# awkrail/svpc

Measured on AMD Instinct MI355X. Metric: train steps/sec (vivt, batch=16, clip_seq=12), higher is better.
Workload: dtype bf16x3; 1 GPU; MODEL_TYPE=vivt train step: N=16 videos/GPU x S=12 clips x Lv=100 frames x F=3072, Lt=22, D=768, H=12, L=6 (enc+step-enc+dec), V=951, A=384, E=10; dropout .1/.1/.4; fwd+bwd+allreduce+clip+BertAdam; mode=bf16x3, global_batch=16, parallelism=dp1, launch=hipGraph replay, gpus_requested=1

## Files before the change

svpc_amd/csrc/layernorm.hip:

```cpp
#include "common.h"
#include <stdlib.h>

template <int W, typename T>
struct VecIO;
template <>
struct VecIO<4, float> {
    static __device__ __forceinline__ void load(const float* p, float* v) {
        float4 t = *reinterpret_cast<const float4*>(p);
        v[0] = t.x; v[1] = t.y; v[2] = t.z; v[3] = t.w;
    }
    static __device__ __forceinline__ void store(float* p, const float* v) {
        *reinterpret_cast<float4*>(p) = make_float4(v[0], v[1], v[2], v[3]);
    }
};
template <>
struct VecIO<1, float> {
    static __device__ __forceinline__ void load(const float* p, float* v) { v[0] = p[0]; }
    static __device__ __forceinline__ void store(float* p, const float* v) { p[0] = v[0]; }
};
typedef __bf16 bf16x4_t __attribute__((ext_vector_type(4)));
template <>
struct VecIO<4, __bf16> {
    static __device__ __forceinline__ void load(const __bf16* p, float* v) {
        bf16x4_t t = *reinterpret_cast<const bf16x4_t*>(p);
        v[0] = (float)t[0]; v[1] = (float)t[1]; v[2] = (float)t[2]; v[3] = (float)t[3];
    }
    static __device__ __forceinline__ void store(__bf16* p, const float* v) {
        bf16x4_t t;
        t[0] = (__bf16)v[0]; t[1] = (__bf16)v[1]; t[2] = (__bf16)v[2]; t[3] = (__bf16)v[3];
        *reinterpret_cast<bf16x4_t*>(p) = t;
    }
};
template <>
struct VecIO<1, __bf16> {
    static __device__ __forceinline__ void load(const __bf16* p, float* v) { v[0] = (float)p[0]; }
    static __device__ __forceinline__ void store(__bf16* p, const float* v) { p[0] = (__bf16)v[0]; }
};

struct split16 { __bf16 v; };
template <>
struct VecIO<4, split16> {
    static __device__ __forceinline__ void load2(const split16* p, int lo, float* v) {
        const bf16x4_t h = *reinterpret_cast<const bf16x4_t*>(p), l = *reinterpret_cast<const bf16x4_t*>(p + lo);
#pragma unroll
        for (int j = 0; j < 4; ++j) v[j] = (float)h[j] + (float)l[j];
    }
    static __device__ __forceinline__ void store2(split16* p, int lo, const float* v) {
        bf16x4_t h, l;
#pragma unroll
        for (int j = 0; j < 4; ++j) { h[j] = (__bf16)v[j]; l[j] = (__bf16)(v[j] - (float)h[j]); }
        *reinterpret_cast<bf16x4_t*>(p) = h;
        *reinterpret_cast<bf16x4_t*>(p + lo) = l;
    }
};
template <>
struct VecIO<1, split16> {
    static __device__ __forceinline__ void load2(const split16* p, int lo, float* v) { v[0] = (float)p[0].v + (float)p[lo].v; }
    static __device__ __forceinline__ void store2(split16* p, int lo, const float* v) {
        const __bf16 h = (__bf16)v[0];
        p[0].v = h; p[lo].v = (__bf16)(v[0] - (float)h);
    }
};
template <typename T> struct IsSplit { static constexpr bool value = false; };
template <> struct IsSplit<split16> { static constexpr bool value = true; };
template <int W, typename T> __device__ __forceinline__ void ln_load(const T* p, int lo, float* v) {
    if constexpr (IsSplit<T>::value) VecIO<W, T>::load2(p, lo, v); else VecIO<W, T>::load(p, v);
}
template <int W, typename T> __device__ __forceinline__ void ln_store(T* p, int lo, const float* v) {
    if constexpr (IsSplit<T>::value) VecIO<W, T>::store2(p, lo, v); else VecIO<W, T>::store(p, v);
}

struct LnArgs {
    const void* x; const int* src_rows; const void* res; const float* gamma; const float* beta;
    void* y; float* mean; float* rstd; int R; int D; float eps;
    float p_pre; uint32_t site_pre; float p_post; uint32_t site_post; const u64* seed;
    const float* add1; int mod1; const float* add2; const int* idx2;
    int ldx, ldr, ldy;
    int lox, lor, loy;
};

template <int NPL, int W, typename TX, typename TY>
__global__ __launch_bounds__(256) void ln_fwd_kernel(LnArgs a) {
    const TX* __restrict__ xp = reinterpret_cast<const TX*>(a.x);
    const TY* __restrict__ rp = reinterpret_cast<const TY*>(a.res);
    TY* __restrict__ yp = reinterpret_cast<TY*>(a.y);
    const int lane = threadIdx.x & 63;
    const int r = __builtin_amdgcn_readfirstlane(blockIdx.x * 4 + (threadIdx.x >> 6));
    if (r >= a.R) return;
    const int D = a.D;
    const size_t xrow = (size_t)(a.src_rows ? a.src_rows[r] : r) * a.ldx;
    const size_t orow = (size_t)r * D;
    const size_t rrow = (size_t)r * a.ldr, yrow = (size_t)r * a.ldy;
    const bool any_drop = (a.p_pre > 0.f) || (a.p_post > 0.f);
    const u64 seed = any_drop ? a.seed[0] : 0ull;
    const float ik_pre = a.p_pre > 0.f ? 1.0f / (1.0f - a.p_pre) : 1.0f;
    const float ik_post = a.p_post > 0.f ? 1.0f / (1.0f - a.p_post) : 1.0f;

    float v[NPL * W];
    float sum = 0.f;
    const bool full = D == NPL * W * 64;
    if (full) {
#pragma unroll
        for (int i = 0; i < NPL; ++i) ln_load<W, TX>(xp + xrow + (lane + 64 * i) * W, a.lox, &v[i * W]);
        if constexpr (NPL * W <= 16) {
            float t[NPL * W];
            if (a.res) {
#pragma unroll
                for (int i = 0; i < NPL; ++i) ln_load<W, TY>(rp + rrow + (lane + 64 * i) * W, a.lor, &t[i * W]);
            }
            if (a.p_pre > 0.f) {
#pragma unroll
                for (int k = 0; k < NPL * W; ++k)
                    v[k] *= drop_scale(seed, a.site_pre, orow + (lane + 64 * (k / W)) * W + (k % W), a.p_pre, ik_pre);
            }
            if (a.res) {
#pragma unroll
                for (int k = 0; k < NPL * W; ++k) v[k] += t[k];
            }
        } else {
            if (a.p_pre > 0.f) {
#pragma unroll
                for (int k = 0; k < NPL * W; ++k)
                    v[k] *= drop_scale(seed, a.site_pre, orow + (lane + 64 * (k / W)) * W + (k % W), a.p_pre, ik_pre);
            }
            if (a.res) {
#pragma unroll
                for (int i = 0; i < NPL; ++i) {
                    float t[W];
                    ln_load<W, TY>(rp + rrow + (lane + 64 * i) * W, a.lor, t);
#pragma unroll
                    for (int j = 0; j < W; ++j) v[i * W + j] += t[j];
                }
            }
        }
#pragma unroll
        for (int k = 0; k < NPL * W; ++k) sum += v[k];
    }
#pragma unroll
    for (int i = 0; i < NPL; ++i) {
        if (full) break;
        const int col = (lane + 64 * i) * W;
        if (col < D) {
            ln_load<W, TX>(xp + xrow + col, a.lox, &v[i * W]);
            if (a.p_pre > 0.f) {
#pragma unroll
                for (int j = 0; j < W; ++j) v[i * W + j] *= drop_scale(seed, a.site_pre, orow + col + j, a.p_pre, ik_pre);
            }
            if (a.res) {
                float t[W];
                ln_load<W, TY>(rp + rrow + col, a.lor, t);
#pragma unroll
                for (int j = 0; j < W; ++j) v[i * W + j] += t[j];
            }
#pragma unroll
            for (int j = 0; j < W; ++j) sum += v[i * W + j];
        }
    }
    const float mean = wave_sum(sum) / (float)D;
    float sq = 0.f;
#pragma unroll
    for (int i = 0; i < NPL; ++i) {
        const int col = (lane + 64 * i) * W;
        if (col < D) {
#pragma unroll
            for (int j = 0; j < W; ++j) {
                float d = v[i * W + j] - mean;
                sq += d * d;
            }
        }
    }
    const float var = wave_sum(sq) / (float)D;
    const float rstd = 1.0f / sqrtf(var + a.eps);
    if (lane == 0) {
        if (a.mean) a.mean[r] = mean;
        if (a.rstd) a.rstd[r] = rstd;
    }
    const size_t a1row = a.add1 ? (size_t)(r % a.mod1) * D : 0;
    const size_t a2row = a.add2 ? (size_t)a.idx2[r] * D : 0;
    if (full) {
        constexpr int CH = NPL < 4 ? NPL : (NPL > 8 ? 2 : 4);
#pragma unroll
        for (int i0 = 0; i0 < NPL; i0 += CH) {
            float g[CH][W], b[CH][W], t1[CH][W], t2[CH][W];
#pragma unroll
            for (int c = 0; c < CH; ++c) {
                if (i0 + c < NPL) {
                    const int col = (lane + 64 * (i0 + c)) * W;
                    VecIO<W, float>::load(a.gamma + col, g[c]);
                    VecIO<W, float>::load(a.beta + col, b[c]);
                }
            }
            if (a.add1) {
#pragma unroll
                for (int c = 0; c < CH; ++c)
                    if (i0 + c < NPL) VecIO<W, float>::load(a.add1 + a1row + (lane + 64 * (i0 + c)) * W, t1[c]);
            }
            if (a.add2) {
#pragma unroll
                for (int c = 0; c < CH; ++c)
                    if (i0 + c < NPL) VecIO<W, float>::load(a.add2 + a2row + (lane + 64 * (i0 + c)) * W, t2[c]);
            }
#pragma unroll
            for (int c = 0; c < CH; ++c) {
                if (i0 + c < NPL) {
                    const int i = i0 + c, col = (lane + 64 * i) * W;
                    float o[W];
#pragma unroll
                    for (int j = 0; j < W; ++j) {
                        float t = (v[i * W + j] - mean) * rstd * g[c][j] + b[c][j];
                        if (a.p_post > 0.f) t *= drop_scale(seed, a.site_post, orow + col + j, a.p_post, ik_post);
                        if (a.add1) t += t1[c][j];
                        if (a.add2) t += t2[c][j];
                        o[j] = t;
                    }
                    ln_store<W, TY>(yp + yrow + col, a.loy, o);
                }
            }
        }
        return;
    }
#pragma unroll
    for (int i = 0; i < NPL; ++i) {
        const int col = (lane + 64 * i) * W;
        if (col < D) {
            float g[W], b[W], o[W];
            VecIO<W, float>::load(a.gamma + col, g);
            VecIO<W, float>::load(a.beta + col, b);
#pragma unroll
            for (int j = 0; j < W; ++j) {
                float t = (v[i * W + j] - mean) * rstd * g[j] + b[j];
                if (a.p_post > 0.f) t *= drop_scale(seed, a.site_post, orow + col + j, a.p_post, ik_post);
                o[j] = t;
            }
            if (a.add1) {
                float t[W];
                VecIO<W, float>::load(a.add1 + a1row + col, t);
#pragma unroll
                for (int j = 0; j < W; ++j) o[j] += t[j];
            }
            if (a.add2) {
                float t[W];
                VecIO<W, float>::load(a.add2 + a2row + col, t);
#pragma unroll
                for (int j = 0; j < W; ++j) o[j] += t[j];
            }
            ln_store<W, TY>(yp + yrow + col, a.loy, o);
        }
    }
}

constexpr int LNW_NPL = 6;
template <typename TX, typename TY>
__global__ __launch_bounds__(256) void ln_fwd_wide_kernel(LnArgs a, int rows_per_wg) {
    __shared__ float gb[2][3072];
    __shared__ float red[2][4];
    const TX* __restrict__ xp = reinterpret_cast<const TX*>(a.x);
    TY* __restrict__ yp = reinterpret_cast<TY*>(a.y);
    const int lane = threadIdx.x & 63, wave = __builtin_amdgcn_readfirstlane(threadIdx.x >> 6);
    const int pair = wave >> 1, half = wave & 1;
    const int D = a.D;
    const int r0 = blockIdx.x * rows_per_wg, r1 = min(a.R, r0 + rows_per_wg);
    const int iters = (r1 - r0 + 1) >> 1;
    const int cbase = (half * LNW_NPL * 64 + lane) * 4;
    const u64 seed = a.p_post > 0.f ? a.seed[0] : 0ull;
    const float ik_post = a.p_post > 0.f ? 1.0f / (1.0f - a.p_post) : 1.0f;
    auto src = [&](int r) { return (size_t)(a.src_rows ? a.src_rows[r] : r) * a.ldx; };
    float v[LNW_NPL * 4], nx[LNW_NPL * 4];
    {
        const size_t xrow = src(min(r0 + pair, r1 - 1));
#pragma unroll
        for (int i = 0; i < LNW_NPL; ++i) ln_load<4, TX>(xp + xrow + cbase + 256 * i, a.lox, &nx[i * 4]);
    }
    for (int c = threadIdx.x * 4; c < D; c += 1024) {
        *reinterpret_cast<float4*>(&gb[0][c]) = *reinterpret_cast<const float4*>(a.gamma + c);
        *reinterpret_cast<float4*>(&gb[1][c]) = *reinterpret_cast<const float4*>(a.beta + c);
    }
    for (int it = 0; it < iters; ++it) {
        const int rr = r0 + 2 * it + pair;
        const bool ok = rr < r1;
        const int r = min(rr, r1 - 1);
#pragma unroll
        for (int k = 0; k < LNW_NPL * 4; ++k) v[k] = nx[k];
        if (it + 1 < iters) {
            const size_t xrow = src(min(rr + 2, r1 - 1));
#pragma unroll
            for (int i = 0; i < LNW_NPL; ++i) ln_load<4, TX>(xp + xrow + cbase + 256 * i, a.lox, &nx[i * 4]);
        }
        float sum = 0.f;
#pragma unroll
        for (int k = 0; k < LNW_NPL * 4; ++k) sum += v[k];
        sum = wave_sum(sum);
        if (lane == 0) red[0][wave] = sum;
        __syncthreads();
        const float mean = (red[0][pair * 2] + red[0][pair * 2 + 1]) / (float)D;
        float sq = 0.f;
#pragma unroll
        for (int k = 0; k < LNW_NPL * 4; ++k) { const float d = v[k] - mean; sq += d * d; }
        sq = wave_sum(sq);
        if (lane == 0) red[1][wave] = sq;
        __syncthreads();
        const float var = (red[1][pair * 2] + red[1][pair * 2 + 1]) / (float)D;
        const float rstd = 1.0f / sqrtf(var + a.eps);
        if (ok && half == 0 && lane == 0) {
            if (a.mean) a.mean[r] = mean;
            if (a.rstd) a.rstd[r] = rstd;
        }
        if (ok) {
            const size_t orow = (size_t)r * D, yrow = (size_t)r * a.ldy;
#pragma unroll
            for (int i = 0; i < LNW_NPL; ++i) {
                const int col = cbase + 256 * i;
                const float4 g = *reinterpret_cast<const float4*>(&gb[0][col]), b = *reinterpret_cast<const float4*>(&gb[1][col]);
                const float gg[4] = {g.x, g.y, g.z, g.w}, bb[4] = {b.x, b.y, b.z, b.w};
                float o[4];
#pragma unroll
                for (int j = 0; j < 4; ++j) {
                    float t = (v[i * 4 + j] - mean) * rstd * gg[j] + bb[j];
                    if (a.p_post > 0.f) t *= drop_scale(seed, a.site_post, orow + col + j, a.p_post, ik_post);
                    o[j] = t;
                }
                ln_store<4, TY>(yp + yrow + col, a.loy, o);
            }
        }
    }
}

struct LnBwdArgs {
    const void* dy; const void* x; const int* src_rows; const void* res; const float* gamma;
    const float* mean; const float* rstd;
    void* dh;
    void* dx;
    float* partial;
    int R; int D;
    float p_pre; uint32_t site_pre; float p_post; uint32_t site_post; const u64* seed;
    int ldx, ldr;
};

template <int NPL, int W, typename TX, typename TY, int RU>
__global__ __launch_bounds__(256, (W == 4 && NPL * W <= 12 && RU == 2) ? 4 : 1) void ln_bwd_kernel(LnBwdArgs a) {
    constexpr bool LACC = W == 4 && NPL * W <= 12 && RU == 2;
    extern __shared__ float smem[];
    const TY* __restrict__ dyp = reinterpret_cast<const TY*>(a.dy);
    const TX* __restrict__ xp = reinterpret_cast<const TX*>(a.x);
    const TY* __restrict__ rp = reinterpret_cast<const TY*>(a.res);
    TY* __restrict__ dhp = reinterpret_cast<TY*>(a.dh);
    TX* __restrict__ dxp = reinterpret_cast<TX*>(a.dx);
    const int lane = threadIdx.x & 63;
    const int wave = __builtin_amdgcn_readfirstlane(threadIdx.x >> 6);
    const int D = a.D;
    const bool any_drop = (a.p_pre > 0.f) || (a.p_post > 0.f);
    const u64 seed = any_drop ? a.seed[0] : 0ull;
    const float ik_pre = a.p_pre > 0.f ? 1.0f / (1.0f - a.p_pre) : 1.0f;
    const float ik_post = a.p_post > 0.f ? 1.0f / (1.0f - a.p_post) : 1.0f;
    const float invD = 1.0f / (float)D;

    float g[LACC ? 1 : NPL * W], accg[LACC ? 1 : NPL * W], accb[LACC ? 1 : NPL * W];
    float* const lg = smem;
    float* const lacc = smem + D + (size_t)wave * 2 * D;
    if constexpr (LACC) {
#pragma unroll
        for (int i = 0; i < NPL; ++i) {
            const int col = (lane + 64 * i) * W;
            if (col < D) {
                *reinterpret_cast<float4*>(lacc + col) = make_float4(0.f, 0.f, 0.f, 0.f);
                *reinterpret_cast<float4*>(lacc + D + col) = make_float4(0.f, 0.f, 0.f, 0.f);
                if (wave == 0) *reinterpret_cast<float4*>(lg + col) = *reinterpret_cast<const float4*>(a.gamma + col);
            }
        }
        __syncthreads();
    } else {
#pragma unroll
        for (int i = 0; i < NPL; ++i) {
            const int col = (lane + 64 * i) * W;
#pragma unroll
            for (int j = 0; j < W; ++j) { accg[i * W + j] = 0.f; accb[i * W + j] = 0.f; g[i * W + j] = 0.f; }
            if (col < D) VecIO<W, float>::load(a.gamma + col, &g[i * W]);
        }
    }
    const int stride = gridDim.x * 4;
    for (int r0 = blockIdx.x * 4 + wave; r0 < a.R; r0 += stride * RU) {
        float h[RU][NPL * W], d[RU][NPL * W];
        float mean[RU], rstd[RU];
        const bool full = D == NPL * W * 64;
#pragma unroll
        for (int u = 0; u < RU; ++u) {
            const int r = r0 + u * stride;
            if (r < a.R) {
                const size_t xrow = (size_t)(a.src_rows ? a.src_rows[r] : r) * a.ldx;
                const size_t orow = (size_t)r * D, rrow = (size_t)r * a.ldr;
                mean[u] = a.mean[r]; rstd[u] = a.rstd[r];
                if (full) {
                    float t[NPL * W];
#pragma unroll
                    for (int i = 0; i < NPL; ++i) VecIO<W, TX>::load(xp + xrow + (lane + 64 * i) * W, &h[u][i * W]);
#pragma unroll
                    for (int i = 0; i < NPL; ++i) VecIO<W, TY>::load(dyp + orow + (lane + 64 * i) * W, &d[u][i * W]);
                    if (a.res) {
#pragma unroll
                        for (int i = 0; i < NPL; ++i) VecIO<W, TY>::load(rp + rrow + (lane + 64 * i) * W, &t[i * W]);
                    }
                    if (a.p_pre > 0.f) {
#pragma unroll
                        for (int i = 0; i < NPL; ++i)
#pragma unroll
                            for (int j = 0; j < W; ++j)
                                h[u][i * W + j] *= drop_scale(seed, a.site_pre, orow + (lane + 64 * i) * W + j, a.p_pre, ik_pre);
                    }
                    if (a.res) {
#pragma unroll
                        for (int k = 0; k < NPL * W; ++k) h[u][k] += t[k];
                    }
                    continue;
                }
#pragma unroll
                for (int i = 0; i < NPL; ++i) {
                    const int col = (lane + 64 * i) * W;
                    if (col < D) {
                        VecIO<W, TX>::load(xp + xrow + col, &h[u][i * W]);
                        VecIO<W, TY>::load(dyp + orow + col, &d[u][i * W]);
                        if (a.res) {
                            float t[W];
                            VecIO<W, TY>::load(rp + rrow + col, t);
                            if (a.p_pre > 0.f) {
#pragma unroll
                                for (int j = 0; j < W; ++j)
                                    h[u][i * W + j] *= drop_scale(seed, a.site_pre, orow + col + j, a.p_pre, ik_pre);
                            }
#pragma unroll
                            for (int j = 0; j < W; ++j) h[u][i * W + j] += t[j];
                        } else if (a.p_pre > 0.f) {
#pragma unroll
                            for (int j = 0; j < W; ++j) h[u][i * W + j] *= drop_scale(seed, a.site_pre, orow + col + j, a.p_pre, ik_pre);
                        }
                    }
                }
            }
        }
#pragma unroll
        for (int u = 0; u < RU; ++u) {
            const int r = r0 + u * stride;
            if (r >= a.R) continue;
            const size_t orow = (size_t)r * D;
            float s1 = 0.f, s2 = 0.f;
#pragma unroll
            for (int i = 0; i < NPL; ++i) {
                const int col = (lane + 64 * i) * W;
                if (col < D) {
                    float gv[W], ag[W], ab[W];
                    if constexpr (LACC) {
                        const float4 t0 = *reinterpret_cast<const float4*>(lg + col), t1 = *reinterpret_cast<const float4*>(lacc + col),
                                     t2 = *reinterpret_cast<const float4*>(lacc + D + col);
                        gv[0] = t0.x; gv[1] = t0.y; gv[2] = t0.z; gv[3] = t0.w;
                        ag[0] = t1.x; ag[1] = t1.y; ag[2] = t1.z; ag[3] = t1.w;
                        ab[0] = t2.x; ab[1] = t2.y; ab[2] = t2.z; ab[3] = t2.w;
                    }
#pragma unroll
                    for (int j = 0; j < W; ++j) {
                        float dy0 = d[u][i * W + j];
                        if (a.p_post > 0.f) dy0 *= drop_scale(seed, a.site_post, orow + col + j, a.p_post, ik_post);
                        const float xhat = (h[u][i * W + j] - mean[u]) * rstd[u];
                        if constexpr (LACC) { ag[j] += dy0 * xhat; ab[j] += dy0; }
                        else { accg[i * W + j] += dy0 * xhat; accb[i * W + j] += dy0; }
                        const float t = dy0 * (LACC ? gv[j] : g[i * W + j]);
                        h[u][i * W + j] = xhat;
                        d[u][i * W + j] = t;
                        s1 += t;
                        s2 += t * xhat;
                    }
                    if constexpr (LACC) {
                        *reinterpret_cast<float4*>(lacc + col) = make_float4(ag[0], ag[1], ag[2], ag[3]);
                        *reinterpret_cast<float4*>(lacc + D + col) = make_float4(ab[0], ab[1], ab[2], ab[3]);
                    }
                }
            }
            if (a.dh || a.dx) {
                s1 = wave_sum(s1) * invD;
                s2 = wave_sum(s2) * invD;
                if (full) {
                    float o[NPL * W];
#pragma unroll
                    for (int k = 0; k < NPL * W; ++k) o[k] = rstd[u] * (d[u][k] - s1 - h[u][k] * s2);
                    if (a.dh) {
#pragma unroll
                        for (int i = 0; i < NPL; ++i) VecIO<W, TY>::store(dhp + orow + (lane + 64 * i) * W, &o[i * W]);
                    }
                    if (a.dx && a.dx != a.dh) {
                        if (a.p_pre > 0.f) {
#pragma unroll
                            for (int k = 0; k < NPL * W; ++k)
                                o[k] *= drop_scale(seed, a.site_pre, orow + (lane + 64 * (k / W)) * W + (k % W), a.p_pre, ik_pre);
                        }
#pragma unroll
                        for (int i = 0; i < NPL; ++i) VecIO<W, TX>::store(dxp + orow + (lane + 64 * i) * W, &o[i * W]);
                    }
                    continue;
                }
#pragma unroll
                for (int i = 0; i < NPL; ++i) {
                    const int col = (lane + 64 * i) * W;
                    if (col < D) {
                        float o[W];
#pragma unroll
                        for (int j = 0; j < W; ++j) o[j] = rstd[u] * (d[u][i * W + j] - s1 - h[u][i * W + j] * s2);
                        if (a.dh) VecIO<W, TY>::store(dhp + orow + col, o);
                        if (a.dx && a.dx != a.dh) {
                            if (a.p_pre > 0.f) {
#pragma unroll
                                for (int j = 0; j < W; ++j) o[j] *= drop_scale(seed, a.site_pre, orow + col + j, a.p_pre, ik_pre);
                            }
                            VecIO<W, TX>::store(dxp + orow + col, o);
                        }
                    }
                }
            }
        }
    }
    if constexpr (LACC) {
        __syncthreads();
        float* out = a.partial + (size_t)blockIdx.x * 2 * D;
        for (int c = threadIdx.x; c < 2 * D; c += 256) {
            float v = smem[D + c];
#pragma unroll
            for (int w = 1; w < 4; ++w) v += smem[D + (size_t)w * 2 * D + c];
            out[c] = v;
        }
        return;
    }
#pragma unroll
    for (int w = 0; w < 4; ++w) {
        if (wave == w) {
#pragma unroll
            for (int i = 0; i < NPL; ++i) {
                const int col = (lane + 64 * i) * W;
                if (col < D) {
#pragma unroll
                    for (int j = 0; j < W; ++j) {
                        if (w == 0) { smem[col + j] = accg[i * W + j]; smem[D + col + j] = accb[i * W + j]; }
                        else { smem[col + j] += accg[i * W + j]; smem[D + col + j] += accb[i * W + j]; }
                    }
                }
            }
        }
        __syncthreads();
    }
    float* out = a.partial + (size_t)blockIdx.x * 2 * D;
    for (int c = threadIdx.x; c < 2 * D; c += 256) out[c] = smem[c];
}

template <typename TX, typename TY>
__global__ __launch_bounds__(256) void ln_param_grad_kernel(LnBwdArgs a, int rows_per_group) {
    __shared__ float red[4][2][256];
    const TY* __restrict__ dyp = reinterpret_cast<const TY*>(a.dy);
    const TX* __restrict__ xp = reinterpret_cast<const TX*>(a.x);
    const TY* __restrict__ rp = reinterpret_cast<const TY*>(a.res);
    const int cg = threadIdx.x & 63, rl = threadIdx.x >> 6, D = a.D;
    const int c0 = (blockIdx.x * 64 + cg) * 4;
    const int group = blockIdx.y;
    const int r0 = group * rows_per_group, r1 = min(a.R, r0 + rows_per_group);
    const bool any_drop = (a.p_pre > 0.f) || (a.p_post > 0.f);
    const u64 seed = any_drop ? a.seed[0] : 0ull;
    const float ik_pre = a.p_pre > 0.f ? 1.0f / (1.0f - a.p_pre) : 1.0f;
    const float ik_post = a.p_post > 0.f ? 1.0f / (1.0f - a.p_post) : 1.0f;
    float ag[4] = {0.f, 0.f, 0.f, 0.f}, ab[4] = {0.f, 0.f, 0.f, 0.f};
    auto one = [&](int r, const float* h, const float* d, const float* t, float mean, float rstd) {
        const size_t orow = (size_t)r * D;
#pragma unroll
        for (int j = 0; j < 4; ++j) {
            float hv = h[j];
            if (a.p_pre > 0.f) hv *= drop_scale(seed, a.site_pre, orow + c0 + j, a.p_pre, ik_pre);
            if (a.res) hv += t[j];
            float dy0 = d[j];
            if (a.p_post > 0.f) dy0 *= drop_scale(seed, a.site_post, orow + c0 + j, a.p_post, ik_post);
            ag[j] += dy0 * (hv - mean) * rstd;
            ab[j] += dy0;
        }
    };
    if (c0 < D) {
        int r = r0 + rl;
        for (; r + 12 < r1; r += 16) {
            float h4[4][4], d4[4][4], t4[4][4];
            float m4[4], s4[4];
#pragma unroll
            for (int q = 0; q < 4; ++q) {
                const int rq = r + 4 * q;
                VecIO<4, TX>::load(xp + (size_t)(a.src_rows ? a.src_rows[rq] : rq) * a.ldx + c0, h4[q]);
                VecIO<4, TY>::load(dyp + (size_t)rq * D + c0, d4[q]);
                if (a.res) VecIO<4, TY>::load(rp + (size_t)rq * a.ldr + c0, t4[q]);
                else { t4[q][0] = t4[q][1] = t4[q][2] = t4[q][3] = 0.f; }
                m4[q] = a.mean[rq]; s4[q] = a.rstd[rq];
            }
#pragma unroll
            for (int q = 0; q < 4; ++q) one(r + 4 * q, h4[q], d4[q], t4[q], m4[q], s4[q]);
        }
        for (; r + 4 < r1; r += 8) {
            const int ra = r, rb = r + 4;
            float ha[4], hb[4], da[4], db[4], ta[4] = {0.f, 0.f, 0.f, 0.f}, tb[4] = {0.f, 0.f, 0.f, 0.f};
            VecIO<4, TX>::load(xp + (size_t)(a.src_rows ? a.src_rows[ra] : ra) * a.ldx + c0, ha);
            VecIO<4, TX>::load(xp + (size_t)(a.src_rows ? a.src_rows[rb] : rb) * a.ldx + c0, hb);
            VecIO<4, TY>::load(dyp + (size_t)ra * D + c0, da);
            VecIO<4, TY>::load(dyp + (size_t)rb * D + c0, db);
            if (a.res) { VecIO<4, TY>::load(rp + (size_t)ra * a.ldr + c0, ta); VecIO<4, TY>::load(rp + (size_t)rb * a.ldr + c0, tb); }
            const float ma = a.mean[ra], sa = a.rstd[ra], mb = a.mean[rb], sb = a.rstd[rb];
            one(ra, ha, da, ta, ma, sa);
            one(rb, hb, db, tb, mb, sb);
        }
        for (; r < r1; r += 4) {
            float h[4], d[4], t[4] = {0.f, 0.f, 0.f, 0.f};
            VecIO<4, TX>::load(xp + (size_t)(a.src_rows ? a.src_rows[r] : r) * a.ldx + c0, h);
            VecIO<4, TY>::load(dyp + (size_t)r * D + c0, d);
            if (a.res) VecIO<4, TY>::load(rp + (size_t)r * a.ldr + c0, t);
            one(r, h, d, t, a.mean[r], a.rstd[r]);
        }
    }
#pragma unroll
    for (int j = 0; j < 4; ++j) { red[rl][0][cg * 4 + j] = ag[j]; red[rl][1][cg * 4 + j] = ab[j]; }
    __syncthreads();
    float* out = a.partial + (size_t)group * 2 * D;
    const int i = threadIdx.x, c = blockIdx.x * 256 + i;
    if (c < D) {
        out[c] = (red[0][0][i] + red[1][0][i]) + (red[2][0][i] + red[3][0][i]);
        out[D + c] = (red[0][1][i] + red[1][1][i]) + (red[2][1][i] + red[3][1][i]);
    }
}

__device__ __forceinline__ float finalize_column(const float* __restrict__ partial, int G, int ncols, int c, int rg, float (*red)[33]) {
    const int cl = threadIdx.x & 31;
    float s = 0.f;
    if (c < ncols) {
        int g = rg;
        for (; g + 224 < G; g += 256) {
            float a[8];
#pragma unroll
            for (int k = 0; k < 8; ++k) a[k] = partial[(size_t)(g + 32 * k) * ncols + c];
#pragma unroll
            for (int k = 0; k < 8; ++k) s += a[k];
        }
        for (; g + 96 < G; g += 128) {
            const float a0 = partial[(size_t)g * ncols + c], a1 = partial[(size_t)(g + 32) * ncols + c];
            const float a2 = partial[(size_t)(g + 64) * ncols + c], a3 = partial[(size_t)(g + 96) * ncols + c];
            s += a0; s += a1; s += a2; s += a3;
        }
        for (; g < G; g += 32) s += partial[(size_t)g * ncols + c];
    }
    red[rg][cl] = s;
    __syncthreads();
    float t = 0.f;
    if (rg == 0) {
        t = red[0][cl];
#pragma unroll
        for (int k = 1; k < 32; ++k) t += red[k][cl];
    }
    return t;
}
__global__ __launch_bounds__(1024) void colsum_finalize_kernel(const float* __restrict__ partial, int G, int ncols,
                                                               float* __restrict__ out, int accumulate) {
    __shared__ float red[32][33];
    const int cl = threadIdx.x & 31, rg = threadIdx.x >> 5;
    const int c = blockIdx.x * 32 + cl;
    const float t = finalize_column(partial, G, ncols, c, rg, red);
    if (rg == 0 && c < ncols) out[c] = accumulate ? out[c] + t : t;
}

__global__ __launch_bounds__(1024) void ln_finalize_kernel(const float* __restrict__ partial, int G, int D, float* __restrict__ dgamma,
                                                           float* __restrict__ dbeta, int accumulate) {
    __shared__ float red[32][33];
    const int cl = threadIdx.x & 31, rg = threadIdx.x >> 5;
    const int c = blockIdx.x * 32 + cl, ncols = 2 * D;
    const float t = finalize_column(partial, G, ncols, c, rg, red);
    if (rg == 0 && c < ncols) {
        float* out = c < D ? dgamma + c : dbeta + (c - D);
        *out = accumulate ? *out + t : t;
    }
}

struct FEntry { const float* partial; float* out0; float* out1; int groups, ncols, split, block0; };
constexpr int FIN_MAX = 64;
struct FArgs { int n; FEntry e[FIN_MAX]; };

__global__ __launch_bounds__(1024) void multi_finalize_kernel(FArgs a) {
    __shared__ float red[32][33];
    int ei = 0;
    while (ei + 1 < a.n && (int)blockIdx.x >= a.e[ei + 1].block0) ++ei;
    const FEntry& en = a.e[ei];
    const int cl = threadIdx.x & 31, rg = threadIdx.x >> 5;
    const int c = ((int)blockIdx.x - en.block0) * 32 + cl;
    const float t = finalize_column(en.partial, en.groups, en.ncols, c, rg, red);
    if (rg == 0 && c < en.ncols) {
        float* out = c < en.split ? en.out0 + c : en.out1 + (c - en.split);
        *out += t;
    }
}

template <int KMAX, typename T>
__global__ __launch_bounds__(256) void bucket_colsum_kernel(const T* __restrict__ x, int ldx, const int* __restrict__ idx,
                                                            int R, int C, int K, int rows_per_chunk, float* __restrict__ partial) {
    const int c = blockIdx.x * 256 + threadIdx.x;
    const int chunk = blockIdx.y;
    const int r0 = chunk * rows_per_chunk;
    const int r1 = min(R, r0 + rows_per_chunk);
    float acc[KMAX];
#pragma unroll
    for (int k = 0; k < KMAX; ++k) acc[k] = 0.f;
    if (c < C) {
        for (int r = r0; r < r1; ++r) {
            const float v = (float)x[(size_t)r * ldx + c];
            const int k = idx ? idx[r] : 0;
#pragma unroll
            for (int kk = 0; kk < KMAX; ++kk) acc[kk] += (kk == k) ? v : 0.f;
        }
#pragma unroll
        for (int k = 0; k < KMAX; ++k)
            if (k < K) partial[((size_t)chunk * K + k) * C + c] = acc[k];
    }
}

template <typename T>
__device__ __forceinline__ void colsum_vec_block(float (*red)[512], const T* __restrict__ x, int ldx, int R, int C, int rows_per_chunk,
                                                 float* __restrict__ partial, int colblock, int chunk) {
    constexpr int V = 16 / sizeof(T);
    typedef float vec16 __attribute__((ext_vector_type(4)));
    typedef __bf16 bf16x8v __attribute__((ext_vector_type(8)));
    const int cg = threadIdx.x & 63, rl = threadIdx.x >> 6;
    const int c0 = (colblock * 64 + cg) * V;
    const int r0 = chunk * rows_per_chunk, r1 = min(R, r0 + rows_per_chunk);
    float acc[V];
#pragma unroll
    for (int j = 0; j < V; ++j) acc[j] = 0.f;
    auto add = [&](const vec16& raw) {
        if (sizeof(T) == 4) {
#pragma unroll
            for (int j = 0; j < 4; ++j) acc[j] += raw[j];
        } else {
            union { vec16 f; bf16x8v h; } u;
            u.f = raw;
#pragma unroll
            for (int j = 0; j < 8; ++j) acc[j % V] += (float)u.h[j];
        }
    };
    if (c0 < C) {
        int r = r0 + rl;
        for (; r + 12 < r1; r += 16) {
            const vec16 a0 = *reinterpret_cast<const vec16*>(x + (size_t)r * ldx + c0);
            const vec16 a1 = *reinterpret_cast<const vec16*>(x + (size_t)(r + 4) * ldx + c0);
            const vec16 a2 = *reinterpret_cast<const vec16*>(x + (size_t)(r + 8) * ldx + c0);
            const vec16 a3 = *reinterpret_cast<const vec16*>(x + (size_t)(r + 12) * ldx + c0);
            add(a0); add(a1); add(a2); add(a3);
        }
        for (; r < r1; r += 4) add(*reinterpret_cast<const vec16*>(x + (size_t)r * ldx + c0));
    }
#pragma unroll
    for (int j = 0; j < V; ++j) red[rl][cg * V + j] = acc[j];
    __syncthreads();
    for (int i = threadIdx.x; i < 64 * V; i += 256) {
        const int c = colblock * 64 * V + i;
        if (c < C) partial[(size_t)chunk * C + c] = (red[0][i] + red[1][i]) + (red[2][i] + red[3][i]);
    }
}

template <typename T>
__global__ __launch_bounds__(256) void colsum_vec_kernel(const T* __restrict__ x, int ldx, int R, int C, int rows_per_chunk,
                                                         float* __restrict__ partial) {
    __shared__ float red[4][512];
    colsum_vec_block<T>(red, x, ldx, R, C, rows_per_chunk, partial, blockIdx.x, blockIdx.y);
}

struct CEntry { const void* x; float* partial; int dt, ldx, R, C, rpc, colblocks, block0; };
constexpr int CSUM_MAX = 48;
struct CArgs { int n; CEntry e[CSUM_MAX]; };
__global__ __launch_bounds__(256) void multi_colsum_kernel(CArgs a) {
    __shared__ float red[4][512];
    int ei = 0;
    while (ei + 1 < a.n && (int)blockIdx.x >= a.e[ei + 1].block0) ++ei;
    const CEntry& en = a.e[ei];
    const int local = blockIdx.x - en.block0;
    const int colblock = local % en.colblocks, chunk = local / en.colblocks;
    if (en.dt == 0) colsum_vec_block<float>(red, (const float*)en.x, en.ldx, en.R, en.C, en.rpc, en.partial, colblock, chunk);
    else colsum_vec_block<__bf16>(red, (const __bf16*)en.x, en.ldx, en.R, en.C, en.rpc, en.partial, colblock, chunk);
}

template <int NPL, int W>
static int launch_ln_fwd(const LnArgs& a, int x_dt, int y_dt, hipStream_t s) {
    const dim3 g(ceil_div(a.R, 4)), b(256);
    if (x_dt == 0 && y_dt == 0) hipLaunchKernelGGL((ln_fwd_kernel<NPL, W, float, float>), g, b, 0, s, a);
    else if (x_dt == 0 && y_dt == 1) hipLaunchKernelGGL((ln_fwd_kernel<NPL, W, float, __bf16>), g, b, 0, s, a);
    else if (x_dt == 1 && y_dt == 1) hipLaunchKernelGGL((ln_fwd_kernel<NPL, W, __bf16, __bf16>), g, b, 0, s, a);
    else if (x_dt == 0 && y_dt == 2) hipLaunchKernelGGL((ln_fwd_kernel<NPL, W, float, split16>), g, b, 0, s, a);
    else if (x_dt == 2 && y_dt == 2) hipLaunchKernelGGL((ln_fwd_kernel<NPL, W, split16, split16>), g, b, 0, s, a);
    else if (x_dt == 2 && y_dt == 0) hipLaunchKernelGGL((ln_fwd_kernel<NPL, W, split16, float>), g, b, 0, s, a);
    else { svpc_set_error("ln_fwd: storage-type combination not instantiated"); return -1; }
    return svpc_check_launch("ln_fwd");
}
template <int NPL, int W>
static int launch_ln_bwd(const LnBwdArgs& a, int G, int x_dt, int y_dt, hipStream_t s) {
    const dim3 g(G), b(256);
    constexpr int RU = (NPL * W <= 16) ? 2 : 1;
    constexpr bool LACC = W == 4 && NPL * W <= 12 && RU == 2;
    static int ru_env = -1;
    if (ru_env < 0) { const char* e = getenv("SVPC_LN_RU"); ru_env = e ? atoi(e) : 0; }
    const size_t lds = (size_t)((LACC && ru_env != 1) ? 9 : 2) * a.D * sizeof(float);
    if (ru_env == 1) {
        if (x_dt == 0 && y_dt == 0) hipLaunchKernelGGL((ln_bwd_kernel<NPL, W, float, float, 1>), g, b, lds, s, a);
        else if (x_dt == 0 && y_dt == 1) hipLaunchKernelGGL((ln_bwd_kernel<NPL, W, float, __bf16, 1>), g, b, lds, s, a);
        else hipLaunchKernelGGL((ln_bwd_kernel<NPL, W, __bf16, __bf16, 1>), g, b, lds, s, a);
        return svpc_check_launch("ln_bwd");
    }
    if (x_dt == 0 && y_dt == 0) hipLaunchKernelGGL((ln_bwd_kernel<NPL, W, float, float, RU>), g, b, lds, s, a);
    else if (x_dt == 0 && y_dt == 1) hipLaunchKernelGGL((ln_bwd_kernel<NPL, W, float, __bf16, RU>), g, b, lds, s, a);
    else hipLaunchKernelGGL((ln_bwd_kernel<NPL, W, __bf16, __bf16, RU>), g, b, lds, s, a);
    return svpc_check_launch("ln_bwd");
}

static bool aligned16(const void* p) { return (((uintptr_t)p) & 15) == 0; }
extern "C" int svpc_ln_param_only_groups(int R);

extern "C" {

int svpc_ln_fwd_s(const void* x, int x_dt, int ldx, int lox, const int* src_rows, const void* res, int ldr, int lor, const float* gamma,
                  const float* beta, void* y, int y_dt, int ldy, int loy, float* mean, float* rstd, int R, int D, float eps, float p_pre,
                  unsigned site_pre, float p_post, unsigned site_post, const u64* seed, const float* add1, int mod1, const float* add2,
                  const int* idx2, hipStream_t stream) {
    if (R == 0) return 0;
    SVPC_REQUIRE(!(x_dt == 1 && y_dt == 0), "ln_fwd: bf16 input with fp32 output is not instantiated");
    if (ldx <= 0) ldx = D;
    if (ldr <= 0) ldr = D;
    if (ldy <= 0) ldy = D;
    SVPC_REQUIRE((x_dt != 2 || (lox >= D && ldx >= lox + D)) && (y_dt != 2 || (loy >= D && ldy >= loy + D && (!res || (lor >= D && ldr >= lor + D)))),
                 "ln_fwd: a split tensor needs its lo plane inside the row, behind the hi plane");
    LnArgs a{x, src_rows, res, gamma, beta, y, mean, rstd, R, D, eps, p_pre, site_pre, p_post, site_post, seed,
             add1, mod1, add2, idx2, ldx, ldr, ldy, lox, lor, loy};
    SVPC_REQUIRE((p_pre <= 0.f && p_post <= 0.f) || seed != nullptr, "ln_fwd: dropout needs a seed pointer");
    const bool vec = (D % 4 == 0) && aligned16(x) && aligned16(y) && aligned16(gamma) && aligned16(beta) &&
                     (!res || aligned16(res)) && (!add1 || aligned16(add1)) && (!add2 || aligned16(add2)) &&
                     ldx % 4 == 0 && ldy % 4 == 0 && ldr % 4 == 0 && lox % 4 == 0 && lor % 4 == 0 && loy % 4 == 0;
    if (vec) {
        if (D <= 256) return launch_ln_fwd<1, 4>(a, x_dt, y_dt, stream);
        static int npl3 = -1;
        if (npl3 < 0) { const char* e = getenv("SVPC_LN_FWD_NPL3"); npl3 = e ? atoi(e) : 1; }
        if (D <= 768 && npl3) return launch_ln_fwd<3, 4>(a, x_dt, y_dt, stream);
        if (D <= 1024) return launch_ln_fwd<4, 4>(a, x_dt, y_dt, stream);
        static int wide = -1;
        if (wide < 0) { const char* e = getenv("SVPC_LN_WIDE"); wide = e ? atoi(e) : 1; }
        if (wide && D == 3072 && x_dt == 0 && !res && p_pre <= 0.f && !add1 && !add2) {
            int rpw = ceil_div(R, 1280);
            rpw += rpw & 1;
            const dim3 g(ceil_div(R, rpw)), b(256);
            if (y_dt == 2) hipLaunchKernelGGL((ln_fwd_wide_kernel<float, split16>), g, b, 0, stream, a, rpw);
            else if (y_dt == 1) hipLaunchKernelGGL((ln_fwd_wide_kernel<float, __bf16>), g, b, 0, stream, a, rpw);
            else hipLaunchKernelGGL((ln_fwd_wide_kernel<float, float>), g, b, 0, stream, a, rpw);
            return svpc_check_launch("ln_fwd_wide");
        }
        if (D <= 3072) return launch_ln_fwd<12, 4>(a, x_dt, y_dt, stream);
        if (D <= 8192) return launch_ln_fwd<32, 4>(a, x_dt, y_dt, stream);
    } else {
        if (D <= 256) return launch_ln_fwd<4, 1>(a, x_dt, y_dt, stream);
        if (D <= 1024) return launch_ln_fwd<16, 1>(a, x_dt, y_dt, stream);
        if (D <= 3072) return launch_ln_fwd<48, 1>(a, x_dt, y_dt, stream);
    }
    svpc_set_error("ln_fwd: row width not supported");
    return -1;
}
int svpc_ln_fwd_t(const void* x, int x_dt, const int* src_rows, const void* res, const float* gamma, const float* beta, void* y,
                  int y_dt, float* mean, float* rstd, int R, int D, float eps, float p_pre, unsigned site_pre, float p_post,
                  unsigned site_post, const u64* seed, const float* add1, int mod1, const float* add2, const int* idx2,
                  hipStream_t stream) {
    SVPC_REQUIRE(x_dt != 2 && y_dt != 2, "ln_fwd_t: split tensors go through svpc_ln_fwd_s");
    return svpc_ln_fwd_s(x, x_dt, D, 0, src_rows, res, D, 0, gamma, beta, y, y_dt, D, 0, mean, rstd, R, D, eps, p_pre, site_pre, p_post,
                         site_post, seed, add1, mod1, add2, idx2, stream);
}
int svpc_ln_fwd(const float* x, const int* src_rows, const float* res, const float* gamma, const float* beta, float* y,
                float* mean, float* rstd, int R, int D, float eps, float p_pre, unsigned site_pre, float p_post,
                unsigned site_post, const u64* seed, const float* add1, int mod1, const float* add2, const int* idx2,
                hipStream_t stream) {
    return svpc_ln_fwd_t(x, 0, src_rows, res, gamma, beta, y, 0, mean, rstd, R, D, eps, p_pre, site_pre, p_post, site_post, seed, add1,
                         mod1, add2, idx2, stream);
}
// ... 178 lines not shown
```

svpc_amd/csrc/optimizer.hip:

```cpp
#include "common.h"

struct TensorMeta { float* p; float* g; float* m; float* v; float* ema; long long n; float wd; int pad; __bf16* shadow; __bf16* shadow_lo; };

constexpr int OPT_CHUNK = 16384;

__global__ __launch_bounds__(256) void opt_sumsq_kernel(const TensorMeta* __restrict__ meta, const int* __restrict__ chunk_tid,
                                                        const long long* __restrict__ chunk_start, float* __restrict__ partial) {
    __shared__ float red[4];
    const int c = blockIdx.x;
    const TensorMeta t = meta[chunk_tid[c]];
    const long long s = chunk_start[c];
    const long long e = s + OPT_CHUNK < t.n ? s + OPT_CHUNK : t.n;
    float acc = 0.f;
    if ((e - s) == OPT_CHUNK && ((((unsigned long long)(t.g + s)) & 15ull) == 0)) {
        const float4* g4 = reinterpret_cast<const float4*>(t.g + s);
        float4 v[OPT_CHUNK / 4 / 256];
#pragma unroll
        for (int k = 0; k < OPT_CHUNK / 4 / 256; ++k) v[k] = g4[threadIdx.x + 256 * k];
#pragma unroll
        for (int k = 0; k < OPT_CHUNK / 4 / 256; ++k) acc += v[k].x * v[k].x + v[k].y * v[k].y + v[k].z * v[k].z + v[k].w * v[k].w;
    } else {
        for (long long i = s + threadIdx.x; i < e; i += 256) { const float g = t.g[i]; acc += g * g; }
    }
    acc = block_sum_256(acc, red);
    if (threadIdx.x == 0) partial[c] = acc;
}
__global__ __launch_bounds__(256) void opt_norms_kernel(const float* __restrict__ partial, const int* __restrict__ tensor_chunk_off,
                                                        int n_tensors, float* __restrict__ norms_sq) {
    __shared__ float red[4];
    float tot = 0.f;
    for (int t = threadIdx.x; t < n_tensors; t += 256) {
        float s = 0.f;
        for (int c = tensor_chunk_off[t]; c < tensor_chunk_off[t + 1]; ++c) s += partial[c];
        norms_sq[t] = s;
        tot += s;
    }
    tot = block_sum_256(tot, red);
    if (threadIdx.x == 0) norms_sq[n_tensors] = tot;
}
__global__ __launch_bounds__(256) void opt_adam_kernel(const TensorMeta* __restrict__ meta, const int* __restrict__ chunk_tid,
                                                       const long long* __restrict__ chunk_start, const float* __restrict__ norms_sq,
                                                       int n_tensors, const float* __restrict__ hyper) {
    const int c = blockIdx.x;
    const int tid = chunk_tid[c];
    const TensorMeta t = meta[tid];
    const float lr = hyper[0], ema_decay = hyper[1], max_g = hyper[2], max_t = hyper[3], b1 = hyper[4], b2 = hyper[5], eps = hyper[6];
    float coef = 1.0f;
    if (max_g > 0.f) coef = fminf(1.0f, max_g / (sqrtf(norms_sq[n_tensors]) + 1e-6f));
    if (max_t > 0.f) {
        const float tn = sqrtf(norms_sq[tid]) * coef;
        coef *= fminf(1.0f, max_t / (tn + 1e-6f));
    }
    const long long s = chunk_start[c];
    const long long e = s + OPT_CHUNK < t.n ? s + OPT_CHUNK : t.n;
    const bool use_ema = t.ema && ema_decay >= 0.f;
    const unsigned long long al = (unsigned long long)(t.g + s) | (unsigned long long)(t.m + s) | (unsigned long long)(t.v + s) |
                                  (unsigned long long)(t.p + s) | (use_ema ? (unsigned long long)(t.ema + s) : 0ull) |
                                  ((t.shadow ? (unsigned long long)(t.shadow + s) : 0ull) << 1) |
                                  ((t.shadow && t.shadow_lo ? (unsigned long long)(t.shadow_lo + s) : 0ull) << 1);
    if ((e - s) == OPT_CHUNK && (al & 15ull) == 0) {
        constexpr int NB = 4, PER = OPT_CHUNK / 4 / 256 / NB;
        float4* __restrict__ g4 = reinterpret_cast<float4*>(t.g + s);
        float4* __restrict__ m4 = reinterpret_cast<float4*>(t.m + s);
        float4* __restrict__ v4 = reinterpret_cast<float4*>(t.v + s);
        float4* __restrict__ p4 = reinterpret_cast<float4*>(t.p + s);
        float4* __restrict__ e4 = reinterpret_cast<float4*>(t.ema + s);
        uint2* __restrict__ sh = reinterpret_cast<uint2*>(t.shadow + s);
        uint2* __restrict__ sl = reinterpret_cast<uint2*>(t.shadow_lo + s);
        for (int b = 0; b < NB; ++b) {
            float4 g[PER], m[PER], v[PER], p[PER], em[PER];
#pragma unroll
            for (int k = 0; k < PER; ++k) {
                const int i = threadIdx.x + 256 * (b * PER + k);
                g[k] = g4[i]; m[k] = m4[i]; v[k] = v4[i]; p[k] = p4[i];
                if (use_ema) em[k] = e4[i];
            }
#pragma unroll
            for (int k = 0; k < PER; ++k) {
                const int i = threadIdx.x + 256 * (b * PER + k);
                float gg[4] = {g[k].x, g[k].y, g[k].z, g[k].w}, mm[4] = {m[k].x, m[k].y, m[k].z, m[k].w};
                float vv[4] = {v[k].x, v[k].y, v[k].z, v[k].w}, pp[4] = {p[k].x, p[k].y, p[k].z, p[k].w};
                float ee[4] = {0.f, 0.f, 0.f, 0.f};
                if (use_ema) { ee[0] = em[k].x; ee[1] = em[k].y; ee[2] = em[k].z; ee[3] = em[k].w; }
                __bf16 hi[4], lo[4];
#pragma unroll
                for (int j = 0; j < 4; ++j) {
                    const float gj = gg[j] * coef;
                    mm[j] = b1 * mm[j] + (1.f - b1) * gj;
                    vv[j] = b2 * vv[j] + (1.f - b2) * gj * gj;
                    float upd = mm[j] / (sqrtf(vv[j]) + eps);
                    if (t.wd > 0.f) upd += t.wd * pp[j];
                    pp[j] -= lr * upd;
                    hi[j] = (__bf16)pp[j];
                    lo[j] = (__bf16)(pp[j] - (float)hi[j]);
                    if (use_ema) ee[j] = (1.f - ema_decay) * pp[j] + ema_decay * ee[j];
                }
                m4[i] = make_float4(mm[0], mm[1], mm[2], mm[3]);
                v4[i] = make_float4(vv[0], vv[1], vv[2], vv[3]);
                p4[i] = make_float4(pp[0], pp[1], pp[2], pp[3]);
                if (t.shadow) {
                    union { __bf16 h[4]; uint2 u; } ph, pl;
#pragma unroll
                    for (int j = 0; j < 4; ++j) { ph.h[j] = hi[j]; pl.h[j] = lo[j]; }
                    sh[i] = ph.u;
                    if (t.shadow_lo) sl[i] = pl.u;
                }
                if (use_ema) e4[i] = make_float4(ee[0], ee[1], ee[2], ee[3]);
            }
        }
        return;
    }
    for (long long i = s + threadIdx.x; i < e; i += 256) {
        const float g = t.g[i] * coef;
        const float m = b1 * t.m[i] + (1.f - b1) * g;
        const float v = b2 * t.v[i] + (1.f - b2) * g * g;
        float p = t.p[i];
        float upd = m / (sqrtf(v) + eps);
        if (t.wd > 0.f) upd += t.wd * p;
        p -= lr * upd;
        t.m[i] = m; t.v[i] = v; t.p[i] = p;
        if (t.shadow) {
            const __bf16 ph = (__bf16)p;
            t.shadow[i] = ph;
            if (t.shadow_lo) t.shadow_lo[i] = (__bf16)(p - (float)ph);
        }
        if (t.ema && ema_decay >= 0.f) t.ema[i] = (1.f - ema_decay) * p + ema_decay * t.ema[i];
    }
}
__global__ __launch_bounds__(256) void opt_zero_kernel(const TensorMeta* __restrict__ meta, const int* __restrict__ chunk_tid,
                                                       const long long* __restrict__ chunk_start) {
    const int c = blockIdx.x;
    const TensorMeta t = meta[chunk_tid[c]];
    const long long s = chunk_start[c];
    const long long e = s + OPT_CHUNK < t.n ? s + OPT_CHUNK : t.n;
    for (long long i = s + threadIdx.x; i < e; i += 256) t.g[i] = 0.f;
}

extern "C" {

int svpc_opt_chunk(void) { return OPT_CHUNK; }
int svpc_opt_meta_bytes(void) { return (int)sizeof(TensorMeta); }

int svpc_opt_step(const void* meta, const int* chunk_tid, const long long* chunk_start, const int* tensor_chunk_off, int n_tensors,
                  int n_chunks, float* partial, float* norms_sq, const float* hyper, hipStream_t s) {
    if (n_chunks == 0) return 0;
    hipLaunchKernelGGL(opt_sumsq_kernel, dim3(n_chunks), dim3(256), 0, s, (const TensorMeta*)meta, chunk_tid, chunk_start, partial);
    int rc = svpc_check_launch("opt_sumsq");
    if (rc) return rc;
    hipLaunchKernelGGL(opt_norms_kernel, dim3(1), dim3(256), 0, s, partial, tensor_chunk_off, n_tensors, norms_sq);
    rc = svpc_check_launch("opt_norms");
    if (rc) return rc;
    hipLaunchKernelGGL(opt_adam_kernel, dim3(n_chunks), dim3(256), 0, s, (const TensorMeta*)meta, chunk_tid, chunk_start, norms_sq,
                       n_tensors, hyper);
    return svpc_check_launch("opt_adam");
}
int svpc_opt_zero_grad(const void* meta, const int* chunk_tid, const long long* chunk_start, int n_chunks, hipStream_t s) {
    if (n_chunks == 0) return 0;
    hipLaunchKernelGGL(opt_zero_kernel, dim3(n_chunks), dim3(256), 0, s, (const TensorMeta*)meta, chunk_tid, chunk_start);
    return svpc_check_launch("opt_zero");
}

}
```

Before: 89.73 steps/s (one step = 16 clip-sequences per GPU; whole-job aggregate).

## Cheaper dropout hashing in LN param-grad; parallelize optimizer norms; nontemporal Adam

In the layernorm parameter-gradient kernel, the per-element dropout hash now uses a row-precomputed key and threshold (RowDrop), so the 64-bit index arithmetic is not redone for every element. The optimizer's per-tensor norm reduction moves from a single 256-thread block to one 64-lane wave per tensor, followed by a separate total kernel. The Adam kernel switches to nontemporal loads and stores and walks its chunks in reverse order, so the chunks touched last by sumsq may still be in cache. Together these add one extra kernel launch and assume the new hash reproduces the old drop_scale masks exactly.

```diff
diff --git a/svpc_amd/csrc/layernorm.hip b/svpc_amd/csrc/layernorm.hip
--- a/svpc_amd/csrc/layernorm.hip
+++ b/svpc_amd/csrc/layernorm.hip
@@ -69,6 +69,16 @@
 template <int W, typename T> __device__ __forceinline__ void ln_store(T* p, int lo, const float* v) {
     if constexpr (IsSplit<T>::value) VecIO<W, T>::store2(p, lo, v); else VecIO<W, T>::store(p, v);
 }
+
+struct RowDrop {
+    uint32_t lo0, hik0, hik1;
+    __device__ __forceinline__ RowDrop(u64 row0)
+        : lo0((uint32_t)row0), hik0((uint32_t)(row0 >> 32) * 0x85EBCA6Bu), hik1(((uint32_t)(row0 >> 32) + 1u) * 0x85EBCA6Bu) {}
+    __device__ __forceinline__ float scale(uint32_t key, uint32_t off, uint32_t thr, float inv_keep) const {
+        const uint32_t lo = lo0 + off;
+        return (svpc_mix32((lo ^ key) + (lo < lo0 ? hik1 : hik0)) >> 16) >= thr ? inv_keep : 0.0f;
+    }
+};
 
 struct LnArgs {
     const void* x; const int* src_rows; const void* res; const float* gamma; const float* beta;
@@ -553,24 +563,26 @@
     const TY* __restrict__ dyp = reinterpret_cast<const TY*>(a.dy);
     const TX* __restrict__ xp = reinterpret_cast<const TX*>(a.x);
     const TY* __restrict__ rp = reinterpret_cast<const TY*>(a.res);
-    const int cg = threadIdx.x & 63, rl = threadIdx.x >> 6, D = a.D;
+    const int cg = threadIdx.x & 63, rl = __builtin_amdgcn_readfirstlane(threadIdx.x >> 6), D = a.D;
     const int c0 = (blockIdx.x * 64 + cg) * 4;
     const int group = blockIdx.y;
     const int r0 = group * rows_per_group, r1 = min(a.R, r0 + rows_per_group);
     const bool any_drop = (a.p_pre > 0.f) || (a.p_post > 0.f);
     const u64 seed = any_drop ? a.seed[0] : 0ull;
+    const uint32_t key_pre = svpc_drop_key(seed, a.site_pre), thr_pre = (uint32_t)(a.p_pre * 65536.0f);
+    const uint32_t key_post = svpc_drop_key(seed, a.site_post), thr_post = (uint32_t)(a.p_post * 65536.0f);
     const float ik_pre = a.p_pre > 0.f ? 1.0f / (1.0f - a.p_pre) : 1.0f;
     const float ik_post = a.p_post > 0.f ? 1.0f / (1.0f - a.p_post) : 1.0f;
     float ag[4] = {0.f, 0.f, 0.f, 0.f}, ab[4] = {0.f, 0.f, 0.f, 0.f};
     auto one = [&](int r, const float* h, const float* d, const float* t, float mean, float rstd) {
-        const size_t orow = (size_t)r * D;
+        const RowDrop rd((u64)r * D);
 #pragma unroll
         for (int j = 0; j < 4; ++j) {
             float hv = h[j];
-            if (a.p_pre > 0.f) hv *= drop_scale(seed, a.site_pre, orow + c0 + j, a.p_pre, ik_pre);
+            if (a.p_pre > 0.f) hv *= rd.scale(key_pre, c0 + j, thr_pre, ik_pre);
             if (a.res) hv += t[j];
             float dy0 = d[j];
-            if (a.p_post > 0.f) dy0 *= drop_scale(seed, a.site_post, orow + c0 + j, a.p_post, ik_post);
+            if (a.p_post > 0.f) dy0 *= rd.scale(key_post, c0 + j, thr_post, ik_post);
             ag[j] += dy0 * (hv - mean) * rstd;
             ab[j] += dy0;
         }
diff --git a/svpc_amd/csrc/optimizer.hip b/svpc_amd/csrc/optimizer.hip
--- a/svpc_amd/csrc/optimizer.hip
+++ b/svpc_amd/csrc/optimizer.hip
@@ -3,6 +3,24 @@
 struct TensorMeta { float* p; float* g; float* m; float* v; float* ema; long long n; float wd; int pad; __bf16* shadow; __bf16* shadow_lo; };
 
 constexpr int OPT_CHUNK = 16384;
+
+#ifndef OPT_ADAM_NT
+#define OPT_ADAM_NT 1
+#endif
+#ifndef OPT_ADAM_REV
+#define OPT_ADAM_REV 1
+#endif
+typedef float opt_f32x4 __attribute__((ext_vector_type(4)));
+__device__ __forceinline__ float4 opt_ld4(const float4* p) {
+    const opt_f32x4* q = reinterpret_cast<const opt_f32x4*>(p);
+    const opt_f32x4 r = OPT_ADAM_NT ? __builtin_nontemporal_load(q) : *q;
+    return make_float4(r[0], r[1], r[2], r[3]);
+}
+__device__ __forceinline__ void opt_st4(float4* p, const float* v) {
+    const opt_f32x4 r = {v[0], v[1], v[2], v[3]};
+    opt_f32x4* q = reinterpret_cast<opt_f32x4*>(p);
+    if (OPT_ADAM_NT) __builtin_nontemporal_store(r, q); else *q = r;
+}
 
 __global__ __launch_bounds__(256) void opt_sumsq_kernel(const TensorMeta* __restrict__ meta, const int* __restrict__ chunk_tid,
                                                         const long long* __restrict__ chunk_start, float* __restrict__ partial) {
@@ -25,23 +43,29 @@
     acc = block_sum_256(acc, red);
     if (threadIdx.x == 0) partial[c] = acc;
 }
-__global__ __launch_bounds__(256) void opt_norms_kernel(const float* __restrict__ partial, const int* __restrict__ tensor_chunk_off,
-                                                        int n_tensors, float* __restrict__ norms_sq) {
+__global__ __launch_bounds__(64) void opt_norms_kernel(const float* __restrict__ partial, const int* __restrict__ tensor_chunk_off,
+                                                       float* __restrict__ norms_sq) {
+    const int t = blockIdx.x, lane = threadIdx.x;
+    const int c0 = tensor_chunk_off[t], c1 = tensor_chunk_off[t + 1];
+    float s = 0.f;
+    for (int c = c0; c < c1; c += 64) {
+        const int n = c1 - c < 64 ? c1 - c : 64;
+        const int v = __float_as_int(lane < n ? partial[c + lane] : 0.f);
+        for (int k = 0; k < n; ++k) s += __int_as_float(__builtin_amdgcn_readlane(v, k));
+    }
+    if (lane == 0) norms_sq[t] = s;
+}
+__global__ __launch_bounds__(256) void opt_total_kernel(int n_tensors, float* __restrict__ norms_sq) {
     __shared__ float red[4];
     float tot = 0.f;
-    for (int t = threadIdx.x; t < n_tensors; t += 256) {
-        float s = 0.f;
-        for (int c = tensor_chunk_off[t]; c < tensor_chunk_off[t + 1]; ++c) s += partial[c];
-        norms_sq[t] = s;
-        tot += s;
-    }
+    for (int t = threadIdx.x; t < n_tensors; t += 256) tot += norms_sq[t];
     tot = block_sum_256(tot, red);
     if (threadIdx.x == 0) norms_sq[n_tensors] = tot;
 }
 __global__ __launch_bounds__(256) void opt_adam_kernel(const TensorMeta* __restrict__ meta, const int* __restrict__ chunk_tid,
                                                        const long long* __restrict__ chunk_start, const float* __restrict__ norms_sq,
                                                        int n_tensors, const float* __restrict__ hyper) {
-    const int c = blockIdx.x;
+    const int c = OPT_ADAM_REV ? (int)(gridDim.x - 1 - blockIdx.x) : (int)blockIdx.x;
     const int tid = chunk_tid[c];
     const TensorMeta t = meta[tid];
     const float lr = hyper[0], ema_decay = hyper[1], max_g = hyper[2], max_t = hyper[3], b1 = hyper[4], b2 = hyper[5], eps = hyper[6];
@@ -72,8 +96,8 @@
 #pragma unroll
             for (int k = 0; k < PER; ++k) {
                 const int i = threadIdx.x + 256 * (b * PER + k);
-                g[k] = g4[i]; m[k] = m4[i]; v[k] = v4[i]; p[k] = p4[i];
-                if (use_ema) em[k] = e4[i];
+                g[k] = opt_ld4(g4 + i); m[k] = opt_ld4(m4 + i); v[k] = opt_ld4(v4 + i); p[k] = opt_ld4(p4 + i);
+                if (use_ema) em[k] = opt_ld4(e4 + i);
             }
 #pragma unroll
             for (int k = 0; k < PER; ++k) {
@@ -95,9 +119,9 @@
                     lo[j] = (__bf16)(pp[j] - (float)hi[j]);
                     if (use_ema) ee[j] = (1.f - ema_decay) * pp[j] + ema_decay * ee[j];
                 }
-                m4[i] = make_float4(mm[0], mm[1], mm[2], mm[3]);
-                v4[i] = make_float4(vv[0], vv[1], vv[2], vv[3]);
-                p4[i] = make_float4(pp[0], pp[1], pp[2], pp[3]);
+                opt_st4(m4 + i, mm);
+                opt_st4(v4 + i, vv);
+                opt_st4(p4 + i, pp);
                 if (t.shadow) {
                     union { __bf16 h[4]; uint2 u; } ph, pl;
 #pragma unroll
@@ -105,7 +129,7 @@
                     sh[i] = ph.u;
                     if (t.shadow_lo) sl[i] = pl.u;
                 }
-                if (use_ema) e4[i] = make_float4(ee[0], ee[1], ee[2], ee[3]);
+                if (use_ema) opt_st4(e4 + i, ee);
             }
         }
         return;
@@ -147,8 +171,11 @@
     hipLaunchKernelGGL(opt_sumsq_kernel, dim3(n_chunks), dim3(256), 0, s, (const TensorMeta*)meta, chunk_tid, chunk_start, partial);
     int rc = svpc_check_launch("opt_sumsq");
     if (rc) return rc;
-    hipLaunchKernelGGL(opt_norms_kernel, dim3(1), dim3(256), 0, s, partial, tensor_chunk_off, n_tensors, norms_sq);
+    hipLaunchKernelGGL(opt_norms_kernel, dim3(n_tensors), dim3(64), 0, s, partial, tensor_chunk_off, norms_sq);
     rc = svpc_check_launch("opt_norms");
+    if (rc) return rc;
+    hipLaunchKernelGGL(opt_total_kernel, dim3(1), dim3(256), 0, s, n_tensors, norms_sq);
+    rc = svpc_check_launch("opt_total");
     if (rc) return rc;
     hipLaunchKernelGGL(opt_adam_kernel, dim3(n_chunks), dim3(256), 0, s, (const TensorMeta*)meta, chunk_tid, chunk_start, norms_sq,
                        n_tensors, hyper);
```

Result: no change. 90.41 steps/s (one step = 16 clip-sequences per GPU; whole-job aggregate), median of 6 (+0.8%).
